# MaxWolf-01/sentinel2-landcover-classification

Hardware: AMD Instinct MI355X
Metric: Sentinel-2 256x256x13 tiles/sec fwd+bwd (higher is better)
Workload: dtype f32

## Files before the change

include/s2k_ops.h:

```cpp
#ifndef S2K_OPS_H
#define S2K_OPS_H

#define S2K_N_T 12
#define S2K_N_N 4
#define S2K_N_D 24
#define S2K_N_F 6

#define S2K_BASE_WS 0
#define S2K_BASE_PARAMS 1
#define S2K_BASE_GRADS 2
#define S2K_BASE_BUFS 3
#define S2K_BASE_X 4
#define S2K_BASE_OUT 5
#define S2K_BASE_DOUT 6
#define S2K_BASE_NOISE 7
#define S2K_BASE_WGS 8
#define S2K_BASE_CONST 9
#define S2K_BASE_Y 10
#define S2K_BASE_AUX 11
#define S2K_BASE_WPACK 12
#define S2K_BASE_DX 13
#define S2K_N_BASES 14

#define S2K_PRO_NONE 0
#define S2K_PRO_AFFINE 1
#define S2K_PRO_SILU 2
#define S2K_PRO_RELU 3
#define S2K_PRO_GELU 4
#define S2K_MODE_CONV 0
#define S2K_MODE_CONVT_SCATTER 1
#define S2K_MODE_GATHER2X2 2
#define S2K_FLAG_SIDE 1
#define S2K_FLAG_JOIN 2
#define S2K_FLAG_BF16 4
#define S2K_FLAG_Q4 16
#define S2K_FLAG_DMA 8
#define S2K_FLAG_RES_GELU_GRAD 32
#define S2K_FLAG_SPLIT 64

#define S2K_OP_MEMSET 1
#define S2K_MEMSET_T_DST 0
#define S2K_MEMSET_N_BYTES 0

#define S2K_OP_AXPY 2
#define S2K_AXPY_T_X 0
#define S2K_AXPY_T_Y 1
#define S2K_AXPY_N_COUNT 0

#define S2K_OP_WEIGHT_PACK 3
#define S2K_WEIGHT_PACK_T_TABLE 0
#define S2K_WEIGHT_PACK_T_SRC 1
#define S2K_WEIGHT_PACK_T_DST 2
#define S2K_WEIGHT_PACK_N_TOTAL 0
#define S2K_WEIGHT_PACK_N_BF16_BASE 1
#define S2K_WEIGHT_PACK_N_Q4_BASE 2
#define S2K_WEIGHT_PACK_N_SPLIT_BASE 3
#define S2K_WEIGHT_PACK_D_N_ENTRIES 0

#define S2K_OP_CONV 4
#define S2K_CONV_T_X1 0
#define S2K_CONV_T_BNV1 1
// ... 732 lines not shown
```

sentinel2-landcover-classification_amd/csrc/common.h:

```cpp
#pragma once
#include <hip/hip_runtime.h>
#include <stdint.h>
#include <stdlib.h>

#include <mutex>
#include <type_traits>

#include "../../include/s2k.h"

namespace s2k {

typedef float f32x16 __attribute__((ext_vector_type(16)));
typedef float f32x4 __attribute__((ext_vector_type(4)));

constexpr int WAVE = 64;
constexpr int NTHREADS = 256;

#ifdef S2K_EXACT_SILU
__device__ __forceinline__ float sigmoid_act(float u) { return 1.0f / (1.0f + expf(-u)); }
#else
__device__ __forceinline__ float sigmoid_act(float u) { return __builtin_amdgcn_rcpf(1.0f + __expf(-u)); }
#endif
__device__ __forceinline__ float silu_f(float u) { return u * sigmoid_act(u); }

// ... 168 lines not shown
        f.bnv[2 * C + c] = mean;
        f.bnv[3 * C + c] = invstd;
    }
}
__device__ __forceinline__ void bn_fold_thread(const BnFold& f, int C, int c, bool writer, float& scale, float& shift) {
    double s = 0.0, q = 0.0;
    for (int r = 0; r < f.nrep; ++r) { s += f.stats[(int64_t)r * 2 * C + c]; q += f.stats[(int64_t)r * 2 * C + C + c]; }
    bn_fold_finish(f, C, c, s, q, writer, scale, shift);
}
__device__ __forceinline__ void bn_fold_wave(const BnFold& f, int C, int c, bool writer, float& scale, float& shift) {
    const int lane = threadIdx.x & 63;
    c = __builtin_amdgcn_readfirstlane(c);
    double s = 0.0, q = 0.0;
    if (f.nrep <= 8) {
        for (int r = 0; r < f.nrep; ++r) { s += f.stats[(int64_t)r * 2 * C + c]; q += f.stats[(int64_t)r * 2 * C + C + c]; }
    } else {
        for (int r = lane; r < f.nrep; r += 64) { s += f.stats[(int64_t)r * 2 * C + c]; q += f.stats[(int64_t)r * 2 * C + C + c]; }
        s = wave_sum_d(s);
        q = wave_sum_d(q);
    }
    bn_fold_finish(f, C, c, s, q, writer && lane == 0, scale, shift);
}

void set_error(const char* fmt, ...);

inline int tune_int(const char* name, int dflt) {
#ifdef S2K_TUNING
    const char* e = getenv(name);
    return e ? atoi(e) : dflt;
#else
    (void)name;
    return dflt;
#endif
}

extern thread_local int g_s2k_variant;

struct PerDeviceOnce {
    std::once_flag flags[64];
    template <typename F>
    void run(F&& f) {
        int d = 0;
        if (hipGetDevice(&d) != hipSuccess || d < 0 || d >= 64) { f(); return; }
        std::call_once(flags[d], f);
    }
};
// ... 38 lines not shown
```

sentinel2-landcover-classification_amd/csrc/dwconv.hip:

```cpp
#include <stdlib.h>

#include <algorithm>

#include "common.h"

namespace s2k {

struct DwP {
    const float* x;
    const float* bnv;
    const float* w;
    const float* dy;
    float* out;
    double* stats;
    int B, C, H, W, K, S, PT, PL, HO, WO, pro, beta, nrep;
    int PPB, RT, bands, IRt, LW;
    int XG, LPP, lwp_shift;
    int vps_shift;
    float inv_xg;
    int bloop, cgroups;
    BnFold fold;
};

__device__ __forceinline__ int chan_of(int64_t plane, int C) { return (int)((uint32_t)plane % (uint32_t)C); }
// ... 954 lines not shown
            }
            if (ok) {
                if (PRO != S2K_PRO_NONE) {
#pragma unroll
                    for (int j = 0; j < 4; ++j) {
                        o[j] *= act_grad(fmaf(xcur[g][j], scale, shift), PRO);
                        s1 += o[j];
                        s2 = fmaf(o[j], (xcur[g][j] - mean) * invstd, s2);
                    }
                }
                *reinterpret_cast<f32x4*>(p.out + off + 4 * li + 256 * g) = f32x4{o[0] + ob[g][0], o[1] + ob[g][1], o[2] + ob[g][2], o[3] + ob[g][3]};
            }
        }
#pragma unroll
        for (int g = 0; g < NG; ++g) { cur[g] = nxt[g]; xcur[g] = xnxt[g]; }
        hcur = hnxt;
    }
    if (p.stats) {
        const double sd = wave_sum_d((double)s1), qd = wave_sum_d((double)s2);
        if (lane == 0) {
            double* st = p.stats + (int64_t)((blockIdx.x + blockIdx.y) % p.nrep) * 2 * p.C;
            atomic_add_d(st + c, sd);
            atomic_add_d(st + p.C + c, qd);
        }
    }
}

template <int K, int PRO, int WO, int RO>
__global__ void __launch_bounds__(NTHREADS) dwconv_dgrad_plane_s2_kernel(const DwP p, int bchunk) {
    constexpr int WI = 2 * WO, PT = (K - 2) / 2;
    constexpr int NB = WO / RO;
    constexpr bool BAND = NB > 1;
    constexpr int GO = RO * WO / 4, LPP = GO, PW = 64 / LPP, XGO = WO / 4;
    constexpr int HT = 1, HB = K == 5 ? 1 : 0;
    constexpr int HGT = BAND ? (HT + HB) * XGO : 0;
    constexpr int TH = RO + HT + HB, TW = WO + 8, TILE = TH * TW;
    constexpr int HWI = WI * WI, HWO = WO * WO;
    static_assert((GO == 64 || GO == 16) && HGT <= 64 && (!BAND || PW == 1), "stride-2 plane geometry");
    extern __shared__ __attribute__((aligned(16))) float smem[];
    const int lane = threadIdx.x & 63, wave = threadIdx.x >> 6;
    const int c = blockIdx.x * 4 + wave;
    if (c >= p.C) return;
    const int n_items = p.B * NB;
    const int i_lo = blockIdx.y * bchunk, i_hi = min(n_items, i_lo + bchunk);
    float scale = 1.0f, shift = 0.0f, mean = 0.0f, invstd = 1.0f;
    if (PRO != S2K_PRO_NONE) { scale = p.bnv[c]; shift = p.bnv[p.C + c]; mean = p.bnv[2 * p.C + c]; invstd = p.bnv[3 * p.C + c]; }
// ... 466 lines not shown
        static const int plane_waves = tune_int("S2K_DW_PLANE_WAVES", 6144);
        int bsplit = std::max(1, std::min(cdiv(n_items, 2 * pw), cdiv(plane_waves, p.C)));
        const int bchunk = cdiv(cdiv(n_items, bsplit), pw) * pw;
        bsplit = cdiv(n_items, bchunk);
        const size_t lds2 = (size_t)4 * 2 * pw * (ro + (p.K == 5 ? 2 : 1)) * (p.WO + 8) * sizeof(float);
        const dim3 grid(cdiv(p.C, 4), bsplit);
        const bool sl = p.pro == S2K_PRO_SILU;
#define DW_DG2(KK, WW, RR) do { \
            if (sl) hipLaunchKernelGGL((dwconv_dgrad_plane_s2_kernel<KK, S2K_PRO_SILU, WW, RR>), grid, dim3(NTHREADS), lds2, c.stream, p, bchunk); \
            else hipLaunchKernelGGL((dwconv_dgrad_plane_s2_kernel<KK, S2K_PRO_NONE, WW, RR>), grid, dim3(NTHREADS), lds2, c.stream, p, bchunk); } while (0)
        if (p.K == 3) {
            if (p.WO == 8) DW_DG2(3, 8, 8); else if (p.WO == 16) DW_DG2(3, 16, 16); else if (p.WO == 32) DW_DG2(3, 32, 8); else DW_DG2(3, 64, 4);
        } else {
            if (p.WO == 8) DW_DG2(5, 8, 8); else if (p.WO == 16) DW_DG2(5, 16, 16); else if (p.WO == 32) DW_DG2(5, 32, 8); else DW_DG2(5, 64, 4);
        }
#undef DW_DG2
        g_s2k_variant = 6;
        return S2K_OK;
    }
    const size_t lds = tile_rows(p, p.H, p.W, irt_dgrad2, p.WO + 2, true, false);
    return p.K == 3 ? launch_dw(dwconv_dgrad_s2_kernel<3>, p, lds, c.stream) : launch_dw(dwconv_dgrad_s2_kernel<5>, p, lds, c.stream);
}

}
```

sentinel2-landcover-classification_amd/csrc/ew.hip:

```cpp
#include "common.h"

namespace s2k {

constexpr int CHUNK = 4096;

template <typename T>
static T* ref_ptr(const Ctx& c, int64_t ref) {
    if (ref < 0) return nullptr;
    const int base = (int)(ref >> 56);
    const int64_t off = ref & ((1ll << 56) - 1);
    if (base >= c.n_bases || c.bases[base] == nullptr) return reinterpret_cast<T*>(1);
    return reinterpret_cast<T*>(static_cast<char*>(c.bases[base]) + off);
}
static bool bad(const void* q) { return q == reinterpret_cast<const void*>(1); }
#define CHECK_PTRS(name, ...)                                                                         \
    do {                                                                                              \
        const void* _ps[] = {__VA_ARGS__};                                                            \
        for (const void* _q : _ps)                                                                    \
            if (bad(_q)) { set_error(name ": tensor references a null base"); return S2K_EFAULT; }    \
    } while (0)

struct Task {
    int64_t plane;
    int start, count;
// ... 1119 lines not shown
    dgamma[c] += (float)s2;
    dbeta[c] += (float)s1;
    const double a = (double)gamma[c] * (double)bnv[3 * C + c];
    coef[c] = (float)a;
    coef[C + c] = (float)(-a * s2 / count);
    coef[2 * C + c] = (float)(-a * s1 / count);
}

int launch_bn_bwd_finalize(const S2kOp& op, const Ctx& c) {
    const double* st2 = ref_ptr<const double>(c, op.t[S2K_BN_BWD_FINALIZE_T_STATS2]);
    const float* gamma = ref_ptr<const float>(c, op.t[S2K_BN_BWD_FINALIZE_T_GAMMA]);
    const float* bnv = ref_ptr<const float>(c, op.t[S2K_BN_BWD_FINALIZE_T_BNV]);
    float* dgamma = ref_ptr<float>(c, op.t[S2K_BN_BWD_FINALIZE_T_DGAMMA]);
    float* dbeta = ref_ptr<float>(c, op.t[S2K_BN_BWD_FINALIZE_T_DBETA]);
    float* coef = ref_ptr<float>(c, op.t[S2K_BN_BWD_FINALIZE_T_COEF]);
    CHECK_PTRS("bn_bwd_finalize", st2, gamma, bnv, dgamma, dbeta, coef);
    const int C = op.d[S2K_BN_BWD_FINALIZE_D_C];
    if (!st2 || !gamma || !bnv || !dgamma || !dbeta || !coef || C <= 0) { set_error("bn_bwd_finalize: bad args"); return S2K_EINVAL; }
    hipLaunchKernelGGL(bn_bwd_finalize_kernel, dim3(cdiv(C, 4)), dim3(256), 0, c.stream, st2, gamma, bnv, dgamma, dbeta, coef, C,
                       (double)op.n[S2K_BN_BWD_FINALIZE_N_COUNT], op.d[S2K_BN_BWD_FINALIZE_D_NREP] > 0 ? op.d[S2K_BN_BWD_FINALIZE_D_NREP] : 1);
    return S2K_OK;
}

struct BnFuse {
    const double* st2;
    const float* gamma;
    float *dgamma, *dbeta;
    double inv_count;
    int nrep;
    const float *mulbc, *addbc;
    float addscale;
    const float* ps;
    int B;
};

__device__ __forceinline__ void bn_fuse_sums(const BnFuse& fz, int C, int c, int lane, double& s1, double& s2) {
    s1 = 0.0; s2 = 0.0;
    if (fz.ps) {
        const int64_t np = (int64_t)fz.B * C;
        for (int b = lane; b < fz.B; b += 64) {
            const int64_t pl = (int64_t)b * C + c;
            const double mul = fz.mulbc ? (double)fz.mulbc[pl] : 1.0, add = fz.addbc ? (double)fz.addbc[pl] * (double)fz.addscale : 0.0;
            s1 += mul * (double)fz.ps[pl] + add * (double)fz.ps[np + pl];
            s2 += mul * (double)fz.ps[2 * np + pl] + add * (double)fz.ps[3 * np + pl];
        }
        s1 = wave_sum_d(s1);
        s2 = wave_sum_d(s2);
    } else if (fz.nrep <= 8) {
        for (int r = 0; r < fz.nrep; ++r) { s1 += fz.st2[(int64_t)r * 2 * C + c]; s2 += fz.st2[(int64_t)r * 2 * C + C + c]; }
    } else {
        for (int r = lane; r < fz.nrep; r += 64) { s1 += fz.st2[(int64_t)r * 2 * C + c]; s2 += fz.st2[(int64_t)r * 2 * C + C + c]; }
        s1 = wave_sum_d(s1);
        s2 = wave_sum_d(s2);
    }
}

__device__ __forceinline__ uint32_t pm_pk_bf16(float lo, float hi) {
    typedef __bf16 b2 __attribute__((ext_vector_type(2)));
    typedef float f2 __attribute__((ext_vector_type(2)));
    f2 v = {lo, hi};
    return __builtin_bit_cast(uint32_t, __builtin_convertvector(v, b2));
}

template <int MODE, bool VEC, bool OUT16 = false>
__global__ void __launch_bounds__(NTHREADS) plane_map_kernel(const float* a, const float* y, const float* bnv, const float* coef,
                                                             const float* noise, float* out, int C, int HW, int64_t nplanes,
                                                             float keep, const BnFuse fz, const BnFold fold = BnFold{}) {
    Task t;
    if (!get_task(HW, nplanes, t)) return;
    const int lane = threadIdx.x & 63;
    const int c = (int)((uint32_t)t.plane % (uint32_t)C);
    const int64_t base = t.plane * HW + t.start;
    float4 av0 = make_float4(0, 0, 0, 0), yv0 = make_float4(0, 0, 0, 0);
    if (VEC && lane < (t.count >> 2)) {
        if (a) av0 = reinterpret_cast<const float4*>(a + base)[lane];
        yv0 = reinterpret_cast<const float4*>(y + base)[lane];
    }
    float k0, k1, k2;
    float gmul = 1.0f, gadd = 0.0f, bscale = 1.0f, bshift = 0.0f;
// ... 414 lines not shown
```

sentinel2-landcover-classification_amd/csrc/s2k_api.hip:

```cpp
#include <cstdarg>
#include <cstdio>
#include <cstring>
#include <mutex>
#include <vector>

#include <stdlib.h>

#include "common.h"

namespace s2k {

static thread_local char g_err[512] = "";
thread_local int g_s2k_variant = 0;

void set_error(const char* fmt, ...) {
    va_list ap;
    va_start(ap, fmt);
    vsnprintf(g_err, sizeof(g_err), fmt, ap);
    va_end(ap);
}

int launch_conv(const S2kOp&, const Ctx&);
int launch_wgrad(const S2kOp&, const Ctx&);
int launch_dwconv_fwd(const S2kOp&, const Ctx&);
// ... 28 lines not shown
int launch_mae_loss_fwd(const S2kOp&, const Ctx&);
int launch_mae_loss_bwd(const S2kOp&, const Ctx&);
int launch_transpose_cl(const S2kOp&, const Ctx&);
int launch_drop_gate(const S2kOp&, const Ctx&);
int launch_confusion(const S2kOp&, const Ctx&);
int launch_tile_prep(const S2kOp&, const Ctx&);
int launch_se_bn_sums(const S2kOp&, const Ctx&);
int launch_se_bn_combine(const S2kOp&, const Ctx&);
int launch_space_to_depth(const S2kOp&, const Ctx&);
int launch_se_fc_wgrad(const S2kOp&, const Ctx&);
int launch_ids_to_dec_idx(const S2kOp&, const Ctx&);
int launch_upsample_zero(const S2kOp&, const Ctx&);
int launch_im2col(const S2kOp&, const Ctx&);
int launch_tile_label_hist(const S2kOp&, const Ctx&);
int launch_tile_moments(const S2kOp&, const Ctx&);
int launch_window_blend(const S2kOp&, const Ctx&);
int launch_seg_stats(const S2kOp&, const Ctx&);
int launch_seg_hist(const S2kOp&, const Ctx&);
int launch_grad_clip(const S2kOp&, const Ctx&);
int launch_tile_radix_hist(const S2kOp&, const Ctx&);
int launch_tile_rank_pick(const S2kOp&, const Ctx&);
int launch_tile_quicklook(const S2kOp&, const Ctx&);
int launch_class_overlay(const S2kOp&, const Ctx&);
int launch_adam(float*, const float*, float*, float*, int64_t, double, double, double, double, double, int, hipStream_t);
int launch_mfma_selftest(const float*, const float*, float*, hipStream_t);

static int launch_memset(const S2kOp& op, const Ctx& c) {
    const int64_t ref = op.t[S2K_MEMSET_T_DST];
    const int64_t bytes = op.n[S2K_MEMSET_N_BYTES];
    if (ref < 0 || bytes <= 0) { set_error("memset: bad args"); return S2K_EINVAL; }
    const int base = (int)(ref >> 56);
    if (base >= c.n_bases || !c.bases[base]) { set_error("memset: null base %d", base); return S2K_EFAULT; }
    char* dst = static_cast<char*>(c.bases[base]) + (ref & ((1ll << 56) - 1));
    if (hipMemsetAsync(dst, 0, (size_t)bytes, c.stream) != hipSuccess) { set_error("memset: hipMemsetAsync failed"); return S2K_EHIP; }
    return S2K_OK;
}

static const char* const kNames[S2K_N_KINDS + 1] = {
    nullptr,
    "MEMSET", "AXPY", "WEIGHT_PACK", "CONV", "WGRAD", "WGRAD_FINALIZE", "DWCONV_FWD", "DWCONV_DGRAD", "DWCONV_WGRAD",
    "BN_FINALIZE", "SE_POOL", "SE_FC", "SE_FC_BWD", "SE_BWD_REDUCE", "BN_BWD_REDUCE", "BN_BWD_FINALIZE", "BN_BWD_APPLY",
    "BN_RESIDUAL", "CHANNEL_SUM", "LOSS_FWD", "LOSS_BWD", "ARGMAX", "CHAN_LN_FWD", "CHAN_LN_BWD", "ACT_BWD", "ACT_FWD",
    "ATTN_FWD", "ATTN_BWD", "MAE_MASK_INDEX", "IDS_TO_DEC_IDX", "TOKEN_GATHER", "TOKEN_SCATTER", "PATCHIFY", "MAE_LOSS_FWD",
    "MAE_LOSS_BWD", "TRANSPOSE_CL", "CONFUSION", "DROP_GATE", "TILE_PREP", "SE_BN_SUMS", "SE_BN_COMBINE", "SPACE_TO_DEPTH",
    "UPSAMPLE_ZERO", "SE_FC_WGRAD", "IM2COL", "TILE_LABEL_HIST", "TILE_MOMENTS", "WINDOW_BLEND",
    "SEG_STATS", "SEG_HIST", "GRAD_CLIP", "TILE_RADIX_HIST", "TILE_RANK_PICK", "TILE_QUICKLOOK", "CLASS_OVERLAY"};
// ... 130 lines not shown

static void release_side_queue(int device, SideQueue* q) {
    if (!q) return;
    std::lock_guard<std::mutex> lk(g_pool_mu);
    g_pool[device].push_back(q);
}

struct DeviceGuard {
    int prev = -1, dev = -1;
    bool switched = false;
    explicit DeviceGuard(hipStream_t st) {
        if (hipGetDevice(&prev) != hipSuccess) prev = -1;
        dev = prev;
        int sd = -1;
        if (st != nullptr && hipStreamGetDevice(st, &sd) == hipSuccess && sd >= 0) dev = sd;
        (void)hipGetLastError();
        if (dev != prev && dev >= 0) switched = hipSetDevice(dev) == hipSuccess;
    }
    ~DeviceGuard() {
        if (switched && prev >= 0) (void)hipSetDevice(prev);
    }
};

int s2k_program_run(const S2kOp* ops, int begin, int end, void* const* bases, int n_bases, void* stream) {
    if (!ops || !bases || begin < 0 || end < begin) { set_error("program_run: bad arguments"); return S2K_EINVAL; }
    hipStream_t main_st = static_cast<hipStream_t>(stream);
    DeviceGuard guard(main_st);
    Ctx c{bases, n_bases, main_st};
    bool any_side = false;
    for (int i = begin; i < end && !any_side; ++i) any_side = (ops[i].flags & S2K_FLAG_SIDE) != 0;
    SideQueue* sq = any_side ? lease_side_queue(guard.dev) : nullptr;
    bool side_busy = false;
    bool main_dirty = true;
    auto join = [&]() {
        if (!side_busy) return;
        (void)hipEventRecord(sq->join, sq->stream);
        (void)hipStreamWaitEvent(main_st, sq->join, 0);
        side_busy = false;
    };
    int rc = S2K_OK;
    for (int i = begin; i < end; ++i) {
        const S2kOp& op = ops[i];
        if ((op.flags & S2K_FLAG_SIDE) && sq) {
            if (main_dirty) {
                (void)hipEventRecord(sq->fork, main_st);
                (void)hipStreamWaitEvent(sq->stream, sq->fork, 0);
                main_dirty = false;
            }
            Ctx cs{bases, n_bases, sq->stream};
            rc = check_launch(dispatch(op, cs), op, i);
            side_busy = true;
        } else {
            if (op.flags & S2K_FLAG_JOIN) join();
            rc = check_launch(dispatch(op, c), op, i);
            main_dirty = true;
        }
        if (rc != S2K_OK) break;
    }
    join();
    release_side_queue(guard.dev, sq);
    return rc;
}

int s2k_op_launch(const S2kOp* op, void* const* bases, int n_bases, void* stream) {
    if (!op || !bases) { set_error("op_launch: bad arguments"); return S2K_EINVAL; }
// ... 20 lines not shown
int s2k_program_profile_variants(const S2kOp* ops, int begin, int end, void* const* bases, int n_bases, void* stream,
                                 float* ms_per_op, int* variant_per_op) {
    float ms[S2K_N_KINDS + 1];
    int cnt[S2K_N_KINDS + 1];
    if (!ms_per_op || !variant_per_op) { set_error("program_profile_variants: bad arguments"); return S2K_EINVAL; }
    return profile_impl(ops, begin, end, bases, n_bases, stream, ms, cnt, ms_per_op, variant_per_op);
}

static int profile_impl(const S2kOp* ops, int begin, int end, void* const* bases, int n_bases, void* stream, float* ms_by_kind,
                        int* launches_by_kind, float* ms_per_op, int* variant_per_op) {
    if (!ops || !bases || !ms_by_kind || !launches_by_kind || begin < 0 || end < begin) {
        set_error("program_profile: bad arguments");
        return S2K_EINVAL;
    }
    hipStream_t st = static_cast<hipStream_t>(stream);
    DeviceGuard guard(st);
    Ctx c{bases, n_bases, st};
    const int n = end - begin;
    hipEvent_t* ev = new hipEvent_t[n + 1];
    for (int i = 0; i <= n; ++i) hipEventCreate(&ev[i]);
    int rc = S2K_OK;
    hipEventRecord(ev[0], st);
    int done = 0;
    for (int i = 0; i < n; ++i) {
        g_s2k_variant = 0;
        rc = check_launch(dispatch(ops[begin + i], c), ops[begin + i], begin + i);
        if (rc != S2K_OK) break;
        if (variant_per_op) variant_per_op[i] = g_s2k_variant;
        hipEventRecord(ev[i + 1], st);
        done = i + 1;
    }
    hipStreamSynchronize(st);
    if (rc == S2K_OK) {
        for (int k = 0; k <= S2K_N_KINDS; ++k) { ms_by_kind[k] = 0.0f; launches_by_kind[k] = 0; }
        for (int i = 0; i < done; ++i) {
            float ms = 0.0f;
            hipEventElapsedTime(&ms, ev[i], ev[i + 1]);
            const int k = ops[begin + i].kind;
            if (ms_per_op) ms_per_op[i] = ms;
            if (k > 0 && k <= S2K_N_KINDS) { ms_by_kind[k] += ms; launches_by_kind[k] += 1; }
        }
    }
    for (int i = 0; i <= n; ++i) hipEventDestroy(ev[i]);
    delete[] ev;
    return rc;
}

int s2k_adam_step(float* p, const float* g, float* m, float* v, int64_t n, double lr, double beta1, double beta2, double eps,
                  double weight_decay, int step, void* stream) {
    DeviceGuard guard(static_cast<hipStream_t>(stream));
    const int rc = launch_adam(p, g, m, v, n, lr, beta1, beta2, eps, weight_decay, step, static_cast<hipStream_t>(stream));
    if (rc != S2K_OK) return rc;
    const hipError_t e = hipGetLastError();
    if (e != hipSuccess) { set_error("adam: %s", hipGetErrorString(e)); return S2K_EHIP; }
    return S2K_OK;
}

int s2k_selftest_mfma(const float* a, const float* b, float* d, void* stream) {
    if (!a || !b || !d) { set_error("selftest: null pointer"); return S2K_EINVAL; }
    DeviceGuard guard(static_cast<hipStream_t>(stream));
    launch_mfma_selftest(a, b, d, static_cast<hipStream_t>(stream));
    const hipError_t e = hipGetLastError();
    if (e != hipSuccess) { set_error("selftest: %s", hipGetErrorString(e)); return S2K_EHIP; }
// ... 5 lines not shown
```

sentinel2-landcover-classification_amd/plan/opdefs.py:

```python
from __future__ import annotations

N_T, N_N, N_D, N_F = 12, 4, 24, 6
OP_BYTES = 8 + 8 * N_T + 8 * N_N + 4 * N_D + 4 * N_F
assert OP_BYTES == 256

BASES = ["WS", "PARAMS", "GRADS", "BUFS", "X", "OUT", "DOUT", "NOISE", "WGS", "CONST", "Y", "AUX", "WPACK", "DX"]
BASE = {n: i for i, n in enumerate(BASES)}

def stats_replicas(C: int) -> int:
    return max(1, min(64, 4096 // max(C, 1)))


PRO_NONE, PRO_AFFINE, PRO_SILU, PRO_RELU, PRO_GELU = 0, 1, 2, 3, 4
ACT_NONE, ACT_SILU, ACT_RELU, ACT_GELU = 0, 2, 3, 4
ACT_MUL = 5
MODE_CONV, MODE_CONVT_SCATTER, MODE_GATHER2X2 = 0, 1, 2
FLAG_SIDE, FLAG_JOIN = 1, 2
FLAG_BF16 = 4
FLAG_Q4 = 16
FLAG_RES_GELU_GRAD = 32
FLAG_SPLIT = 64
FLAG_DMA = 8

FOLD_T, FOLD_N, FOLD_D, FOLD_F = ["FSTATS", "FGAMMA", "FBETA", "FRM", "FRV"], ["FCOUNT"], ["FNREP"], ["FEPS", "FMOM"]
FOLD_KINDS = ("DWCONV_FWD", "SE_POOL", "BN_RESIDUAL")

OPS: dict[str, tuple[list[str], list[str], list[str], list[str]]] = {
    "MEMSET": (["DST"], ["BYTES"], [], []),
    "AXPY": (["X", "Y"], ["COUNT"], [], []),
    "WEIGHT_PACK": (["TABLE", "SRC", "DST"], ["TOTAL", "BF16_BASE", "Q4_BASE", "SPLIT_BASE"], ["N_ENTRIES"], []),
    "CONV": (["X1", "BNV1", "GATE1", "X2", "BNV2", "WT", "BIAS", "Y", "STATS", "RES", "SCRATCH", "WTB"], [],
             ["B", "C1", "C2", "H", "W", "M", "KH", "KW", "STRIDE", "PAD_T", "PAD_L", "HO", "WO",
              "PRO1", "PRO2", "MODE", "W_SM", "W_SK", "W_ST", "FLIP", "BETA", "YC", "NREP", "X1_BF16"], []),
    "WGRAD": (["P", "BNVP", "GATEP", "Q", "BNVQ", "GATEQ", "WGS"], [],
              ["B", "M", "C", "CTOT", "H", "W", "KH", "KW", "STRIDE", "PAD_T", "PAD_L", "HO", "WO",
               "PROP", "PROQ", "MODE", "P_BF16"], []),
    "WGRAD_FINALIZE": (["TABLE", "WGS", "GRADS"], ["TOTAL"], ["N_ENTRIES"], []),
    "DWCONV_FWD": (["X", "BNV", "WT", "Y", "STATS"] + FOLD_T, FOLD_N,
                   ["B", "C", "H", "W", "K", "STRIDE", "PAD_T", "PAD_L", "HO", "WO", "PRO", "NREP"] + FOLD_D, FOLD_F),
    "DWCONV_DGRAD": (["DY", "WT", "XRAW", "BNV", "G", "STATS2"], [],
                     ["B", "C", "H", "W", "K", "STRIDE", "PAD_T", "PAD_L", "HO", "WO", "PRO", "BETA", "NREP"], []),
    "DWCONV_WGRAD": (["DY", "X", "BNV", "DW"], [],
                     ["B", "C", "H", "W", "K", "STRIDE", "PAD_T", "PAD_L", "HO", "WO", "PRO"], []),
    "BN_FINALIZE": (["STATS", "GAMMA", "BETA", "RM", "RV", "BNV"], ["COUNT"], ["C", "TRAIN", "NREP"], ["EPS", "MOM"]),
    "SE_POOL": (["Y", "BNV", "POOL"] + FOLD_T, FOLD_N, ["B", "C", "HW", "PRO"] + FOLD_D, FOLD_F),
# ... 95 lines not shown
```

sentinel2-landcover-classification_amd/plan/unet_plan.py:

```python
from __future__ import annotations

import math
from dataclasses import dataclass, field

from . import opdefs as D
from .program import Arena, Program, TRef

CAT_SIZES = {
    "b0": [592, 296, 152, 80], "b1": [592, 296, 152, 80], "b2": [600, 304, 152, 80],
    "b3": [608, 304, 160, 88], "b4": [624, 312, 160, 88], "b5": [640, 320, 168, 88],
    "b6": [656, 328, 168, 96], "b7": [672, 336, 176, 96],
}


@dataclass
class BlockSpec:
    kernel: int
    stride: int
    cin: int
    cout: int
    expand: int
    se: int
    residual: bool

# ... 726 lines not shown
                continue
            if kind in ("WGRAD", "DWCONV_WGRAD", "CHANNEL_SUM", "SE_FC_WGRAD"):
                f["_flags"] = D.FLAG_SIDE
            elif kind == "WGRAD_FINALIZE":
                f["_flags"] = D.FLAG_SIDE if finalize_on_side else D.FLAG_JOIN
        side_stream_hazards(p.bwd)
        n_before = len(p.bwd.ops)
        attach_q4()
        if not bwd_pack_in_fwd:
            pack_op(p.bwd, p.pack_rows["bwd"])
        if len(p.bwd.ops) > n_before:
            segments = [(a + 1 if a else 0, b + 1, lo, hi) for (a, b, lo, hi) in segments]
        bwd = p.bwd
    else:
        attach_q4()
    pack_op(p.fwd, p.pack_rows["fwd"])
    if bwd_pack_in_fwd:
        pack_op(p.fwd, p.pack_rows["bwd"], D.FLAG_SIDE)
    attach_splitk_scratch()
    if getattr(p, "bf16", False):
        mark_bf16(p, bwd)
    if getattr(p, "split", False):
        mark_split(p, bwd)
    return segments, bwd


def side_stream_hazards(prog: Program) -> int:
    def ranges(f, names):
        out = []
        for k in names:
            v = f.get(k)
            if isinstance(v, TRef):
                out.append((v.base, v.off, v.off + v.nbytes))
        return out

    pending: list = []
    added = 0
    for kind, f in prog.ops:
        flags = f.get("_flags", 0)
        t_names = D.OPS[kind][0]
        writes = D.WRITES.get(kind, tuple(t_names))
        if flags & D.FLAG_SIDE:
            pending.extend(ranges(f, [k for k in t_names if k not in writes]))
            continue
        if flags & D.FLAG_JOIN:
            pending.clear()
# ... 61 lines not shown
    from . import split as SP

    base = (p.wpack.mark() + 255) // 256 * 256
    keep = D.FLAG_Q4 | D.FLAG_RES_GELU_GRAD | D.FLAG_DMA | D.FLAG_BF16
    packs, split_convs = [], 0
    for prog in (p.fwd, bwd):
        if prog is None:
            continue
        for kind, f in prog.ops:
            if kind == "WEIGHT_PACK":
                packs.append(f)
            elif kind == "CONV" and isinstance(f.get("WT"), TRef) and f["WT"].base == D.BASE["WPACK"] and not (f.get("_flags", 0) & keep) \
                    and f["WT"].shape[0] == -(-(f["C1"] + f["C2"]) // 64) * 64 * f["KH"] * f["KW"] and SP.routed(kind, f):
                f["_flags"] = f.get("_flags", 0) | D.FLAG_SPLIT
                f["WTB"] = TRef(D.BASE["WPACK"], base + 3 * (f["WT"].off // 2), f["WT"].shape, "i16", "split:" + f["WT"].name)
                split_convs += 1
            elif kind == "WGRAD" and not (f.get("_flags", 0) & D.FLAG_BF16) and SP.routed(kind, f):
                f["_flags"] = f.get("_flags", 0) | D.FLAG_SPLIT
    if not split_convs:
        return
    for f in packs:
        f["SPLIT_BASE"] = base
    p.wpack.top = base + 3 * ((base + 1) // 2) + 256


def fold_bn_finalize(prog: Program) -> int:
    if tune("S2K_FOLD_BN", "1") != "1":
        return 0
    ops = prog.ops
    folded = 0
    i = 0
    while i < len(ops):
        kind, f = ops[i]
        if kind != "BN_FINALIZE" or not f.get("TRAIN") or f.get("_flags"):
            i += 1
            continue
        bnv = f["BNV"]
        touched = {t.ref for k in ("BNV", "RM", "RV", "STATS") if isinstance(t := f.get(k), TRef)}
        target = None
        for j in range(i + 1, len(ops)):
            k2, f2 = ops[j]
            refs = {v.ref for v in f2.values() if isinstance(v, TRef)}
            if not (refs & touched):
                continue
            if (k2 in D.FOLD_KINDS and isinstance(f2.get("BNV"), TRef) and f2["BNV"].ref == bnv.ref and f2.get("FSTATS") is None
                    and f2.get("C") == f["C"] and f2.get("PRO", 1) and len(refs & touched) == 1 and not f2.get("_flags")):
# ... 115 lines not shown
```

Baseline: 988.7.

## Fuse BN-backward, depthwise wgrad/dgrad and second BN-backward into one chain kernel

Adds a dw_bwd_chain kernel that runs four backward ops (BN backward apply with SiLU, depthwise conv weight grad, depthwise conv data grad, BN backward apply) in one launch per channel, for 8x8 and 16x16 stride-1 planes. The planner tags matching op sequences with a new CHAIN flag, and the runtime dispatches the fused kernel when the pattern checks pass. The aim is to avoid writing and re-reading dy and g through global memory, cut launch count, and skip the intermediate stats buffer. The trade-offs are one block per channel, which limits parallelism at small C, a second pass over g, and reductions that are serial within a block.

```diff
diff --git a/include/s2k_ops.h b/include/s2k_ops.h
--- a/include/s2k_ops.h
+++ b/include/s2k_ops.h
@@ -37,6 +37,7 @@
 #define S2K_FLAG_DMA 8
 #define S2K_FLAG_RES_GELU_GRAD 32
 #define S2K_FLAG_SPLIT 64
+#define S2K_FLAG_CHAIN 128
 
 #define S2K_OP_MEMSET 1
 #define S2K_MEMSET_T_DST 0
diff --git a/sentinel2-landcover-classification_amd/csrc/common.h b/sentinel2-landcover-classification_amd/csrc/common.h
--- a/sentinel2-landcover-classification_amd/csrc/common.h
+++ b/sentinel2-landcover-classification_amd/csrc/common.h
@@ -214,6 +214,39 @@
     bn_fold_finish(f, C, c, s, q, writer && lane == 0, scale, shift);
 }
 
+struct BnFuse {
+    const double* st2;
+    const float* gamma;
+    float *dgamma, *dbeta;
+    double inv_count;
+    int nrep;
+    const float *mulbc, *addbc;
+    float addscale;
+    const float* ps;
+    int B;
+};
+
+__device__ __forceinline__ void bn_fuse_sums(const BnFuse& fz, int C, int c, int lane, double& s1, double& s2) {
+    s1 = 0.0; s2 = 0.0;
+    if (fz.ps) {
+        const int64_t np = (int64_t)fz.B * C;
+        for (int b = lane; b < fz.B; b += 64) {
+            const int64_t pl = (int64_t)b * C + c;
+            const double mul = fz.mulbc ? (double)fz.mulbc[pl] : 1.0, add = fz.addbc ? (double)fz.addbc[pl] * (double)fz.addscale : 0.0;
+            s1 += mul * (double)fz.ps[pl] + add * (double)fz.ps[np + pl];
+            s2 += mul * (double)fz.ps[2 * np + pl] + add * (double)fz.ps[3 * np + pl];
+        }
+        s1 = wave_sum_d(s1);
+        s2 = wave_sum_d(s2);
+    } else if (fz.nrep <= 8) {
+        for (int r = 0; r < fz.nrep; ++r) { s1 += fz.st2[(int64_t)r * 2 * C + c]; s2 += fz.st2[(int64_t)r * 2 * C + C + c]; }
+    } else {
+        for (int r = lane; r < fz.nrep; r += 64) { s1 += fz.st2[(int64_t)r * 2 * C + c]; s2 += fz.st2[(int64_t)r * 2 * C + C + c]; }
+        s1 = wave_sum_d(s1);
+        s2 = wave_sum_d(s2);
+    }
+}
+
 void set_error(const char* fmt, ...);
 
 inline int tune_int(const char* name, int dflt) {
diff --git a/sentinel2-landcover-classification_amd/csrc/dwconv.hip b/sentinel2-landcover-classification_amd/csrc/dwconv.hip
--- a/sentinel2-landcover-classification_amd/csrc/dwconv.hip
+++ b/sentinel2-landcover-classification_amd/csrc/dwconv.hip
@@ -1000,6 +1000,171 @@
             double* st = p.stats + (int64_t)((blockIdx.x + blockIdx.y) % p.nrep) * 2 * p.C;
             atomic_add_d(st + c, sd);
             atomic_add_d(st + p.C + c, qd);
+        }
+    }
+}
+
+struct DwChainP {
+    const float *d, *ydw, *bnv1, *mulbc, *addbc, *ps, *gamma1;
+    float *dy, *dgamma1, *dbeta1;
+    const float *x, *bnv2, *w, *gamma2;
+    float *dw, *g, *dgamma2, *dbeta2;
+    double inv_count1, inv_count2;
+    float addscale;
+    int B, C;
+};
+
+template <int K, int W>
+__global__ void __launch_bounds__(NTHREADS) dw_bwd_chain_kernel(const DwChainP p) {
+    constexpr int PADK = (K - 1) / 2, KK = K * K;
+    constexpr int GPP = W * W / 4, LPP = GPP > 64 ? 64 : GPP, PW = 64 / LPP, XGW = W / 4;
+    constexpr int TH = W + K - 1, TW = W + 8, TILE = TH * TW, HW = W * W;
+    constexpr int WAVE_TILES = 2 * 2 * PW * TILE;
+    static_assert(GPP == 64 || GPP == 16, "8 x 8 or 16 x 16 planes");
+    static_assert((4 * WAVE_TILES) % 4 == 0, "the reduction scratch behind the tiles stays 16-byte aligned");
+    extern __shared__ __attribute__((aligned(16))) float smem[];
+    const int lane = threadIdx.x & 63, wave = threadIdx.x >> 6;
+    const int c = blockIdx.x;
+    const int B = p.B, C = p.C;
+    const int sub = lane / LPP, li = lane % LPP;
+    const int r = li / XGW, xg = li % XGW;
+    const int64_t bstride = (int64_t)C * HW;
+    const int64_t loff = (int64_t)c * HW + 4 * li;
+    const f32x4 zero = {0.f, 0.f, 0.f, 0.f};
+    const int b_first = wave * PW + sub;
+    f32x4 dcur, ycur, xcur;
+    float mcur, acur;
+    {
+        const int bc = min(b_first, B - 1);
+        const int64_t off = (int64_t)bc * bstride + loff;
+        dcur = *reinterpret_cast<const f32x4*>(p.d + off);
+        ycur = *reinterpret_cast<const f32x4*>(p.ydw + off);
+        xcur = *reinterpret_cast<const f32x4*>(p.x + off);
+        mcur = p.mulbc[(int64_t)bc * C + c];
+        acur = p.addbc[(int64_t)bc * C + c];
+    }
+    BnFuse fz{};
+    fz.mulbc = p.mulbc; fz.addbc = p.addbc; fz.addscale = p.addscale; fz.ps = p.ps; fz.B = B;
+    double s1d, s2d;
+    bn_fuse_sums(fz, C, c, lane, s1d, s2d);
+    const float bscale1 = p.bnv1[c], bshift1 = p.bnv1[C + c];
+    float k0, k1, k2;
+    {
+        const float mean = p.bnv1[2 * C + c], invstd = p.bnv1[3 * C + c];
+        const double aa = (double)p.gamma1[c] * (double)invstd;
+        const float A = (float)aa, Bq = (float)(-aa * s2d * p.inv_count1), Cq = (float)(-aa * s1d * p.inv_count1);
+        k0 = A; k1 = Bq * invstd; k2 = Cq - Bq * invstd * mean;
+        if (threadIdx.x == 0) {
+            p.dgamma1[c] += (float)s2d;
+            p.dbeta1[c] += (float)s1d;
+        }
+    }
+    const float scale2 = p.bnv2[c], shift2 = p.bnv2[C + c], mean2 = p.bnv2[2 * C + c], invstd2 = p.bnv2[3 * C + c];
+    float wk[KK];
+#pragma unroll
+    for (int i = 0; i < KK; ++i) wk[i] = p.w[c * KK + (KK - 1 - i)];
+    float* tiles = smem + wave * WAVE_TILES;
+    for (int i = lane; i < WAVE_TILES / 4; i += 64) reinterpret_cast<f32x4*>(tiles)[i] = zero;
+    float acc[KK];
+#pragma unroll
+    for (int i = 0; i < KK; ++i) acc[i] = 0.0f;
+    float s1 = 0.0f, s2 = 0.0f;
+    int buf = 0;
+    for (int b = b_first; b - sub < B; b += 4 * PW, buf ^= 1) {
+        const bool ok = b < B;
+        f32x4 dnxt, ynxt, xnxt;
+        float mnxt, anxt;
+        {
+            const int bc = min(b + 4 * PW, B - 1);
+            const int64_t off = (int64_t)bc * bstride + loff;
+            dnxt = *reinterpret_cast<const f32x4*>(p.d + off);
+            ynxt = *reinterpret_cast<const f32x4*>(p.ydw + off);
+            xnxt = *reinterpret_cast<const f32x4*>(p.x + off);
+            mnxt = p.mulbc[(int64_t)bc * C + c];
+            anxt = p.addbc[(int64_t)bc * C + c];
+        }
+        const float gadd = acur * p.addscale;
+        f32x4 dy1, av;
+#pragma unroll
+        for (int j = 0; j < 4; ++j) {
+            const float g1 = fmaf(dcur[j], mcur, gadd) * act_grad(fmaf(ycur[j], bscale1, bshift1), S2K_PRO_SILU);
+            dy1[j] = fmaf(k0, g1, fmaf(k1, ycur[j], k2));
+            av[j] = apply_pro_c<S2K_PRO_SILU>(xcur[j], scale2, shift2);
+        }
+        if (!ok) { dy1 = zero; av = zero; }
+        else *reinterpret_cast<f32x4*>(p.dy + (int64_t)b * bstride + loff) = dy1;
+        float* td = tiles + ((buf * 2 + 0) * PW + sub) * TILE;
+        float* ta = tiles + ((buf * 2 + 1) * PW + sub) * TILE;
+        *reinterpret_cast<f32x4*>(td + (r + PADK) * TW + 4 + 4 * xg) = dy1;
+        *reinterpret_cast<f32x4*>(ta + (r + PADK) * TW + 4 + 4 * xg) = av;
+        __builtin_amdgcn_wave_barrier();
+        float o[4] = {0.f, 0.f, 0.f, 0.f};
+        const float* d0 = td + r * TW + 4 * xg;
+        const float* a0 = ta + r * TW + 4 * xg;
+#pragma unroll
+        for (int ky = 0; ky < K; ++ky) {
+            float win[12];
+            read_window<3>(a0 + ky * TW, win);
+#pragma unroll
+            for (int kx = 0; kx < K; ++kx)
+#pragma unroll
+                for (int j = 0; j < 4; ++j) acc[ky * K + kx] = fmaf(dy1[j], win[4 - PADK + j + kx], acc[ky * K + kx]);
+            read_window<3>(d0 + ky * TW, win);
+#pragma unroll
+            for (int kx = 0; kx < K; ++kx)
+#pragma unroll
+                for (int j = 0; j < 4; ++j) o[j] = fmaf(wk[ky * K + kx], win[4 - PADK + j + kx], o[j]);
+        }
+        if (ok) {
+#pragma unroll
+            for (int j = 0; j < 4; ++j) {
+                o[j] *= act_grad(fmaf(xcur[j], scale2, shift2), S2K_PRO_SILU);
+                s1 += o[j];
+                s2 = fmaf(o[j], (xcur[j] - mean2) * invstd2, s2);
+            }
+            *reinterpret_cast<f32x4*>(p.g + (int64_t)b * bstride + loff) = f32x4{o[0], o[1], o[2], o[3]};
+        }
+        dcur = dnxt; ycur = ynxt; xcur = xnxt; mcur = mnxt; acur = anxt;
+    }
+    double* red_s = reinterpret_cast<double*>(smem + 4 * WAVE_TILES);
+    float* red_t = smem + 4 * WAVE_TILES + 16;
+    {
+        const double sd = wave_sum_d((double)s1), qd = wave_sum_d((double)s2);
+        if (lane == 0) { red_s[wave * 2] = sd; red_s[wave * 2 + 1] = qd; }
+#pragma unroll
+        for (int i = 0; i < KK; ++i) {
+            const float v = wave_sum(acc[i]);
+            if (lane == 0) red_t[wave * KK + i] = v;
+        }
+    }
+    __syncthreads();
+    if ((int)threadIdx.x < KK) p.dw[c * KK + threadIdx.x] += (red_t[threadIdx.x] + red_t[KK + threadIdx.x]) + (red_t[2 * KK + threadIdx.x] + red_t[3 * KK + threadIdx.x]);
+    {
+        const double t1 = (red_s[0] + red_s[2]) + (red_s[4] + red_s[6]), t2 = (red_s[1] + red_s[3]) + (red_s[5] + red_s[7]);
+        const double aa = (double)p.gamma2[c] * (double)invstd2;
+        const float A = (float)aa, Bq = (float)(-aa * t2 * p.inv_count2), Cq = (float)(-aa * t1 * p.inv_count2);
+        k0 = A; k1 = Bq * invstd2; k2 = Cq - Bq * invstd2 * mean2;
+        if (threadIdx.x == 0) {
+            p.dgamma2[c] += (float)t2;
+            p.dbeta2[c] += (float)t1;
+        }
+    }
+    for (int b = b_first; b - sub < B; b += 8 * PW) {
+        const int b1 = b + 4 * PW;
+        const int64_t off0 = (int64_t)min(b, B - 1) * bstride + loff, off1 = (int64_t)min(b1, B - 1) * bstride + loff;
+        const f32x4 g0 = *reinterpret_cast<const f32x4*>(p.g + off0), x0 = *reinterpret_cast<const f32x4*>(p.x + off0);
+        const f32x4 g1 = *reinterpret_cast<const f32x4*>(p.g + off1), x1 = *reinterpret_cast<const f32x4*>(p.x + off1);
+        if (b < B) {
+            f32x4 v;
+#pragma unroll
+            for (int j = 0; j < 4; ++j) v[j] = fmaf(k0, g0[j], fmaf(k1, x0[j], k2));
+            *reinterpret_cast<f32x4*>(p.g + off0) = v;
+        }
+        if (b1 < B) {
+            f32x4 v;
+#pragma unroll
+            for (int j = 0; j < 4; ++j) v[j] = fmaf(k0, g1[j], fmaf(k1, x1[j], k2));
+            *reinterpret_cast<f32x4*>(p.g + off1) = v;
         }
     }
 }
@@ -1512,4 +1677,49 @@
     return p.K == 3 ? launch_dw(dwconv_dgrad_s2_kernel<3>, p, lds, c.stream) : launch_dw(dwconv_dgrad_s2_kernel<5>, p, lds, c.stream);
 }
 
-}
+int launch_dw_bwd_chain(const S2kOp* o, const Ctx& c) {
+    const S2kOp &a1 = o[0], &wg = o[1], &dg = o[2], &a2 = o[3];
+    DwChainP p{};
+    p.d = ref_ptr<const float>(c, a1.t[S2K_BN_BWD_APPLY_T_GP]);
+    p.dy = ref_ptr<float>(c, a1.t[S2K_BN_BWD_APPLY_T_DY]);
+    p.ydw = ref_ptr<const float>(c, a1.t[S2K_BN_BWD_APPLY_T_Y]);
+    p.bnv1 = ref_ptr<const float>(c, a1.t[S2K_BN_BWD_APPLY_T_BNV]);
+    p.mulbc = ref_ptr<const float>(c, a1.t[S2K_BN_BWD_APPLY_T_MULBC]);
+    p.addbc = ref_ptr<const float>(c, a1.t[S2K_BN_BWD_APPLY_T_ADDBC]);
+    p.ps = ref_ptr<const float>(c, a1.t[S2K_BN_BWD_APPLY_T_PS]);
+    p.gamma1 = ref_ptr<const float>(c, a1.t[S2K_BN_BWD_APPLY_T_GAMMA]);
+    p.dgamma1 = ref_ptr<float>(c, a1.t[S2K_BN_BWD_APPLY_T_DGAMMA]);
+    p.dbeta1 = ref_ptr<float>(c, a1.t[S2K_BN_BWD_APPLY_T_DBETA]);
+    p.x = ref_ptr<const float>(c, dg.t[S2K_DWCONV_DGRAD_T_XRAW]);
+    p.bnv2 = ref_ptr<const float>(c, dg.t[S2K_DWCONV_DGRAD_T_BNV]);
+    p.w = ref_ptr<const float>(c, dg.t[S2K_DWCONV_DGRAD_T_WT]);
+    p.dw = ref_ptr<float>(c, wg.t[S2K_DWCONV_WGRAD_T_DW]);
+    p.g = ref_ptr<float>(c, dg.t[S2K_DWCONV_DGRAD_T_G]);
+    p.gamma2 = ref_ptr<const float>(c, a2.t[S2K_BN_BWD_APPLY_T_GAMMA]);
+    p.dgamma2 = ref_ptr<float>(c, a2.t[S2K_BN_BWD_APPLY_T_DGAMMA]);
+    p.dbeta2 = ref_ptr<float>(c, a2.t[S2K_BN_BWD_APPLY_T_DBETA]);
+    const void* all[] = {p.d, p.dy, p.ydw, p.bnv1, p.mulbc, p.addbc, p.ps, p.gamma1, p.dgamma1, p.dbeta1, p.x, p.bnv2, p.w, p.dw, p.g, p.gamma2,
+                         p.dgamma2, p.dbeta2};
+    for (const void* q : all) {
+        if (bad(q)) { set_error("dw_bwd_chain: null base"); return S2K_EFAULT; }
+        if (!q) { set_error("dw_bwd_chain: missing tensor"); return S2K_EINVAL; }
+    }
+    p.B = dg.d[0]; p.C = dg.d[1];
+    const int W = dg.d[3], K = dg.d[4];
+    p.inv_count1 = 1.0 / (double)a1.n[S2K_BN_BWD_APPLY_N_COUNT];
+    p.inv_count2 = 1.0 / (double)a2.n[S2K_BN_BWD_APPLY_N_COUNT];
+    p.addscale = a1.f[S2K_BN_BWD_APPLY_F_ADDSCALE];
+    const int pw = W == 8 ? 4 : 1;
+    const size_t lds = ((size_t)4 * 2 * 2 * pw * (W + K - 1) * (W + 8) + 16 + 4 * K * K) * sizeof(float);
+    if (lds > 64 * 1024) { set_error("dw_bwd_chain: tile too large (%zu B)", lds); return S2K_EINVAL; }
+    const dim3 grid(p.C);
+    if (K == 3 && W == 8) hipLaunchKernelGGL((dw_bwd_chain_kernel<3, 8>), grid, dim3(NTHREADS), lds, c.stream, p);
+    else if (K == 3 && W == 16) hipLaunchKernelGGL((dw_bwd_chain_kernel<3, 16>), grid, dim3(NTHREADS), lds, c.stream, p);
+    else if (K == 5 && W == 8) hipLaunchKernelGGL((dw_bwd_chain_kernel<5, 8>), grid, dim3(NTHREADS), lds, c.stream, p);
+    else if (K == 5 && W == 16) hipLaunchKernelGGL((dw_bwd_chain_kernel<5, 16>), grid, dim3(NTHREADS), lds, c.stream, p);
+    else { set_error("dw_bwd_chain: unsupported plane %d, k %d", W, K); return S2K_EINVAL; }
+    g_s2k_variant = 10;
+    return S2K_OK;
+}
+
+}
diff --git a/sentinel2-landcover-classification_amd/csrc/ew.hip b/sentinel2-landcover-classification_amd/csrc/ew.hip
--- a/sentinel2-landcover-classification_amd/csrc/ew.hip
+++ b/sentinel2-landcover-classification_amd/csrc/ew.hip
@@ -1165,39 +1165,6 @@
     return S2K_OK;
 }
 
-struct BnFuse {
-    const double* st2;
-    const float* gamma;
-    float *dgamma, *dbeta;
-    double inv_count;
-    int nrep;
-    const float *mulbc, *addbc;
-    float addscale;
-    const float* ps;
-    int B;
-};
-
-__device__ __forceinline__ void bn_fuse_sums(const BnFuse& fz, int C, int c, int lane, double& s1, double& s2) {
-    s1 = 0.0; s2 = 0.0;
-    if (fz.ps) {
-        const int64_t np = (int64_t)fz.B * C;
-        for (int b = lane; b < fz.B; b += 64) {
-            const int64_t pl = (int64_t)b * C + c;
-            const double mul = fz.mulbc ? (double)fz.mulbc[pl] : 1.0, add = fz.addbc ? (double)fz.addbc[pl] * (double)fz.addscale : 0.0;
-            s1 += mul * (double)fz.ps[pl] + add * (double)fz.ps[np + pl];
-            s2 += mul * (double)fz.ps[2 * np + pl] + add * (double)fz.ps[3 * np + pl];
-        }
-        s1 = wave_sum_d(s1);
-        s2 = wave_sum_d(s2);
-    } else if (fz.nrep <= 8) {
-        for (int r = 0; r < fz.nrep; ++r) { s1 += fz.st2[(int64_t)r * 2 * C + c]; s2 += fz.st2[(int64_t)r * 2 * C + C + c]; }
-    } else {
-        for (int r = lane; r < fz.nrep; r += 64) { s1 += fz.st2[(int64_t)r * 2 * C + c]; s2 += fz.st2[(int64_t)r * 2 * C + C + c]; }
-        s1 = wave_sum_d(s1);
-        s2 = wave_sum_d(s2);
-    }
-}
-
 __device__ __forceinline__ uint32_t pm_pk_bf16(float lo, float hi) {
     typedef __bf16 b2 __attribute__((ext_vector_type(2)));
     typedef float f2 __attribute__((ext_vector_type(2)));
diff --git a/sentinel2-landcover-classification_amd/csrc/s2k_api.hip b/sentinel2-landcover-classification_amd/csrc/s2k_api.hip
--- a/sentinel2-landcover-classification_amd/csrc/s2k_api.hip
+++ b/sentinel2-landcover-classification_amd/csrc/s2k_api.hip
@@ -74,6 +74,7 @@
 int launch_tile_rank_pick(const S2kOp&, const Ctx&);
 int launch_tile_quicklook(const S2kOp&, const Ctx&);
 int launch_class_overlay(const S2kOp&, const Ctx&);
+int launch_dw_bwd_chain(const S2kOp*, const Ctx&);
 int launch_adam(float*, const float*, float*, float*, int64_t, double, double, double, double, double, int, hipStream_t);
 int launch_mfma_selftest(const float*, const float*, float*, hipStream_t);
 
@@ -250,6 +251,37 @@
     }
 };
 
+static int try_dw_chain(const S2kOp* ops, int i, int end, const Ctx& c, int* rc) {
+    if (!(ops[i].flags & S2K_FLAG_CHAIN) || i + 3 >= end) return 0;
+    const S2kOp &a1 = ops[i], &wg = ops[i + 1], &dg = ops[i + 2], &a2 = ops[i + 3];
+    if (a1.kind != S2K_OP_BN_BWD_APPLY || wg.kind != S2K_OP_DWCONV_WGRAD || dg.kind != S2K_OP_DWCONV_DGRAD || a2.kind != S2K_OP_BN_BWD_APPLY) return 0;
+    if ((a1.flags | wg.flags | dg.flags | a2.flags) & (S2K_FLAG_BF16 | S2K_FLAG_SPLIT)) return 0;
+    const int64_t dy = a1.t[S2K_BN_BWD_APPLY_T_DY], x = dg.t[S2K_DWCONV_DGRAD_T_XRAW], g = dg.t[S2K_DWCONV_DGRAD_T_G];
+    if (dy < 0 || a1.t[S2K_BN_BWD_APPLY_T_GP] != dy || a1.t[S2K_BN_BWD_APPLY_T_COEF] >= 0 || a1.t[S2K_BN_BWD_APPLY_T_PS] < 0 ||
+        a1.t[S2K_BN_BWD_APPLY_T_MULBC] < 0 || a1.t[S2K_BN_BWD_APPLY_T_ADDBC] < 0 || a1.d[S2K_BN_BWD_APPLY_D_ACT] != S2K_PRO_SILU ||
+        a1.d[S2K_BN_BWD_APPLY_D_EVAL] || a1.d[S2K_BN_BWD_APPLY_D_OUT_BF16] || a1.n[S2K_BN_BWD_APPLY_N_COUNT] <= 0) return 0;
+    if (wg.t[S2K_DWCONV_WGRAD_T_DY] != dy || dg.t[S2K_DWCONV_DGRAD_T_DY] != dy || x < 0 || wg.t[S2K_DWCONV_WGRAD_T_X] != x ||
+        dg.t[S2K_DWCONV_DGRAD_T_BNV] < 0 || wg.t[S2K_DWCONV_WGRAD_T_BNV] != dg.t[S2K_DWCONV_DGRAD_T_BNV] || g < 0 || g == dy || g == x ||
+        dg.t[S2K_DWCONV_DGRAD_T_STATS2] < 0) return 0;
+    for (int k = 0; k <= 10; ++k)
+        if (wg.d[k] != dg.d[k]) return 0;
+    const int B = dg.d[0], C = dg.d[1], H = dg.d[2], W = dg.d[3], K = dg.d[4];
+    if (B <= 0 || C <= 0 || H != W || (W != 8 && W != 16) || (K != 3 && K != 5) || dg.d[5] != 1 || dg.d[6] != (K - 1) / 2 || dg.d[7] != (K - 1) / 2 ||
+        dg.d[8] != H || dg.d[9] != W || dg.d[10] != S2K_PRO_SILU || dg.d[S2K_DWCONV_DGRAD_D_BETA] != 0) return 0;
+    if ((int64_t)B * C * H * W * 4 >= 0x7ffffff0ll) return 0;
+    if (a2.t[S2K_BN_BWD_APPLY_T_GP] != g || a2.t[S2K_BN_BWD_APPLY_T_DY] != g || a2.t[S2K_BN_BWD_APPLY_T_Y] != x ||
+        a2.t[S2K_BN_BWD_APPLY_T_BNV] != dg.t[S2K_DWCONV_DGRAD_T_BNV] || a2.t[S2K_BN_BWD_APPLY_T_STATS2] != dg.t[S2K_DWCONV_DGRAD_T_STATS2] ||
+        a2.t[S2K_BN_BWD_APPLY_T_COEF] >= 0 || a2.t[S2K_BN_BWD_APPLY_T_PS] >= 0 || a2.t[S2K_BN_BWD_APPLY_T_MULBC] >= 0 ||
+        a2.t[S2K_BN_BWD_APPLY_T_ADDBC] >= 0 || a2.d[S2K_BN_BWD_APPLY_D_ACT] != S2K_PRO_NONE || a2.d[S2K_BN_BWD_APPLY_D_EVAL] ||
+        a2.d[S2K_BN_BWD_APPLY_D_OUT_BF16] || a2.n[S2K_BN_BWD_APPLY_N_COUNT] <= 0) return 0;
+    const int HW = H * W;
+    if (a1.d[S2K_BN_BWD_APPLY_D_B] != B || a1.d[S2K_BN_BWD_APPLY_D_C] != C || a1.d[S2K_BN_BWD_APPLY_D_HW] != HW ||
+        a2.d[S2K_BN_BWD_APPLY_D_B] != B || a2.d[S2K_BN_BWD_APPLY_D_C] != C || a2.d[S2K_BN_BWD_APPLY_D_HW] != HW) return 0;
+    g_s2k_variant = 0;
+    *rc = check_launch(launch_dw_bwd_chain(&ops[i], c), ops[i], i);
+    return 4;
+}
+
 int s2k_program_run(const S2kOp* ops, int begin, int end, void* const* bases, int n_bases, void* stream) {
     if (!ops || !bases || begin < 0 || end < begin) { set_error("program_run: bad arguments"); return S2K_EINVAL; }
     hipStream_t main_st = static_cast<hipStream_t>(stream);
@@ -269,6 +301,16 @@
     int rc = S2K_OK;
     for (int i = begin; i < end; ++i) {
         const S2kOp& op = ops[i];
+        if ((op.flags & S2K_FLAG_CHAIN) && i + 3 < end) {
+            if ((op.flags | ops[i + 1].flags | ops[i + 2].flags | ops[i + 3].flags) & S2K_FLAG_JOIN) join();
+            const int used = try_dw_chain(ops, i, end, c, &rc);
+            if (used) {
+                main_dirty = true;
+                if (rc != S2K_OK) break;
+                i += used - 1;
+                continue;
+            }
+        }
         if ((op.flags & S2K_FLAG_SIDE) && sq) {
             if (main_dirty) {
                 (void)hipEventRecord(sq->fork, main_st);
@@ -335,12 +377,18 @@
     int rc = S2K_OK;
     hipEventRecord(ev[0], st);
     int done = 0;
+    std::vector<char> fused(n, 0);
     for (int i = 0; i < n; ++i) {
         g_s2k_variant = 0;
-        rc = check_launch(dispatch(ops[begin + i], c), ops[begin + i], begin + i);
+        const int used = try_dw_chain(ops, begin + i, end, c, &rc);
+        if (!used) rc = check_launch(dispatch(ops[begin + i], c), ops[begin + i], begin + i);
         if (rc != S2K_OK) break;
-        if (variant_per_op) variant_per_op[i] = g_s2k_variant;
-        hipEventRecord(ev[i + 1], st);
+        for (int k = 0; k < (used ? used : 1); ++k) {
+            if (variant_per_op) variant_per_op[i + k] = g_s2k_variant;
+            hipEventRecord(ev[i + k + 1], st);
+            if (k) fused[i + k] = 1;
+        }
+        if (used) i += used - 1;
         done = i + 1;
     }
     hipStreamSynchronize(st);
@@ -348,10 +396,10 @@
         for (int k = 0; k <= S2K_N_KINDS; ++k) { ms_by_kind[k] = 0.0f; launches_by_kind[k] = 0; }
         for (int i = 0; i < done; ++i) {
             float ms = 0.0f;
-            hipEventElapsedTime(&ms, ev[i], ev[i + 1]);
+            if (!fused[i]) hipEventElapsedTime(&ms, ev[i], ev[i + 1]);
             const int k = ops[begin + i].kind;
             if (ms_per_op) ms_per_op[i] = ms;
-            if (k > 0 && k <= S2K_N_KINDS) { ms_by_kind[k] += ms; launches_by_kind[k] += 1; }
+            if (k > 0 && k <= S2K_N_KINDS && !fused[i]) { ms_by_kind[k] += ms; launches_by_kind[k] += 1; }
         }
     }
     for (int i = 0; i <= n; ++i) hipEventDestroy(ev[i]);
diff --git a/sentinel2-landcover-classification_amd/plan/opdefs.py b/sentinel2-landcover-classification_amd/plan/opdefs.py
--- a/sentinel2-landcover-classification_amd/plan/opdefs.py
+++ b/sentinel2-landcover-classification_amd/plan/opdefs.py
@@ -21,6 +21,7 @@
 FLAG_RES_GELU_GRAD = 32
 FLAG_SPLIT = 64
 FLAG_DMA = 8
+FLAG_CHAIN = 128
 
 FOLD_T, FOLD_N, FOLD_D, FOLD_F = ["FSTATS", "FGAMMA", "FBETA", "FRM", "FRV"], ["FCOUNT"], ["FNREP"], ["FEPS", "FMOM"]
 FOLD_KINDS = ("DWCONV_FWD", "SE_POOL", "BN_RESIDUAL")
diff --git a/sentinel2-landcover-classification_amd/plan/unet_plan.py b/sentinel2-landcover-classification_amd/plan/unet_plan.py
--- a/sentinel2-landcover-classification_amd/plan/unet_plan.py
+++ b/sentinel2-landcover-classification_amd/plan/unet_plan.py
@@ -772,6 +772,7 @@
         mark_bf16(p, bwd)
     if getattr(p, "split", False):
         mark_split(p, bwd)
+    mark_dw_chain(p, bwd, segments)
     return segments, bwd
 
 
@@ -879,6 +880,59 @@
     for f in packs:
         f["SPLIT_BASE"] = base
     p.wpack.top = base + 3 * ((base + 1) // 2) + 256
+
+
+def mark_dw_chain(p: "_P", bwd, segments=None) -> int:
+    if bwd is None or tune("S2K_DW_CHAIN", "1") != "1":
+        return 0
+    ops = bwd.ops
+    seg_end = {}
+    for (a, b, _lo, _hi) in (segments or [(0, len(ops), 0, 0)]):
+        for i in range(a, b):
+            seg_end[i] = b
+    bad_flags = D.FLAG_BF16 | D.FLAG_SPLIT
+    kinds = ("BN_BWD_APPLY", "DWCONV_WGRAD", "DWCONV_DGRAD", "BN_BWD_APPLY")
+
+    def same(a, b):
+        return isinstance(a, TRef) and isinstance(b, TRef) and a.ref == b.ref
+
+    marked = 0
+    for i in range(len(ops) - 3):
+        if tuple(k for k, _ in ops[i:i + 4]) != kinds or seg_end.get(i, 0) < i + 4:
+            continue
+        a1, wg, dg, a2 = (f for _, f in ops[i:i + 4])
+        if any(f.get("_flags", 0) & bad_flags for f in (a1, wg, dg, a2)):
+            continue
+        dy, x, g, st2 = a1.get("DY"), dg.get("XRAW"), dg.get("G"), dg.get("STATS2")
+        if not (same(a1.get("GP"), dy) and same(wg.get("DY"), dy) and same(dg.get("DY"), dy)
+                and same(wg.get("X"), x) and same(a2.get("Y"), x) and same(a2.get("GP"), g) and same(a2.get("DY"), g)
+                and same(a2.get("STATS2"), st2) and same(wg.get("BNV"), dg.get("BNV")) and same(a2.get("BNV"), dg.get("BNV"))):
+            continue
+        if not (a1.get("ACT") == D.ACT_SILU and isinstance(a1.get("PS"), TRef) and isinstance(a1.get("MULBC"), TRef)
+                and isinstance(a1.get("ADDBC"), TRef) and a1.get("COEF") is None and not a1.get("EVAL") and not a1.get("OUT_BF16")):
+            continue
+        if not (a2.get("COEF") is None and not a2.get("ACT") and a2.get("PS") is None and a2.get("MULBC") is None
+                and a2.get("ADDBC") is None and not a2.get("EVAL") and not a2.get("OUT_BF16")):
+            continue
+        geo = ("B", "C", "H", "W", "K", "STRIDE", "PAD_T", "PAD_L", "HO", "WO", "PRO")
+        K, W = dg["K"], dg["W"]
+        if not (all(wg[k] == dg[k] for k in geo) and dg["STRIDE"] == 1 and dg["PRO"] == D.PRO_SILU and not dg.get("BETA")
+                and dg["H"] == W and W in (8, 16) and K in (3, 5) and dg["HO"] == W and dg["WO"] == W
+                and dg["PAD_T"] == (K - 1) // 2 and dg["PAD_L"] == (K - 1) // 2):
+            continue
+        if not all(f["B"] == dg["B"] and f["C"] == dg["C"] and f["HW"] == W * W for f in (a1, a2)):
+            continue
+        dead = [(t.base, t.off, t.off + t.nbytes) for t in (st2,)]
+        live = False
+        for _k2, f2 in ops[i + 4:]:
+            for v in f2.values():
+                if isinstance(v, TRef) and any(v.base == b and v.off < hi and lo < v.off + v.nbytes for (b, lo, hi) in dead):
+                    live = True
+        if live:
+            continue
+        a1["_flags"] = a1.get("_flags", 0) | D.FLAG_CHAIN
+        marked += 1
+    return marked
 
 
 def fold_bn_finalize(prog: Program) -> int:
```

New measurement: 999.7, median of 6. 1.01x the previous value.
